# Bissmella/Small-object-detection-transformers

Measured on AMD Instinct MI355X. Metric: images/sec (1024x1024 RGB+IR) train fwd+bwd, higher is better.
Workload: dtype bf16; 1 GPU; SRyolo_MF.yaml (model.yaml graph), batch 8/GPU @ 1024x1024 RGB+IR, fwd + hand-written bwd + fused SGD-nesterov/weight-decay + EMA step, loss = YOLOv5 ComputeLoss (CIoU + BCE, device kernels), 32 synthetic boxes/image, random-init weights; global_batch=8, parallelism=dp1

## Files before the change

small-object-detection-transformers_amd/csrc/head.hip:

```cpp
#include "common.h"
#include "../../include/sodt_hip.h"

namespace {

__global__ void bn_finalize_kernel(const double* __restrict__ stats, float* __restrict__ mr, float* __restrict__ rmean,
                                   float* __restrict__ rvar, long count, int C, float eps, float momentum) {
  const int c = blockIdx.x * blockDim.x + threadIdx.x;
  if (c >= C) return;
  if (stats) {
    double s1 = 0.0, s2 = 0.0;
    for (int r = 0; r < SODT_STATS_REPL; ++r) { s1 += stats[(size_t)r * 2 * C + c]; s2 += stats[(size_t)r * 2 * C + C + c]; }
    const double mean = s1 / (double)count;
    double var = s2 / (double)count - mean * mean;
    if (var < 0.0) var = 0.0;
    mr[c] = (float)mean;
    mr[C + c] = (float)(1.0 / sqrt(var + (double)eps));
    if (rmean) {
      const double unb = count > 1 ? var * (double)count / (double)(count - 1) : var;
      rmean[c] = (1.0f - momentum) * rmean[c] + momentum * (float)mean;
      rvar[c] = (1.0f - momentum) * rvar[c] + momentum * (float)unb;
    }
  } else {
    mr[c] = rmean[c];
    mr[C + c] = rsqrtf(rvar[c] + eps);
  }
}

__global__ void bn_affine_kernel(const float* __restrict__ mr, const float* __restrict__ gamma,
                                 const float* __restrict__ beta, float* __restrict__ scale, float* __restrict__ shift, int C) {
  const int c = blockIdx.x * blockDim.x + threadIdx.x;
  if (c >= C) return;
  const float s = gamma[c] * mr[C + c];
  scale[c] = s;
  shift[c] = beta[c] - mr[c] * s;
}

template <typename T>
__global__ __launch_bounds__(256) void bn_silu_fwd_kernel(const T* __restrict__ z, const float* __restrict__ mr,
                                                         const float* __restrict__ gamma, const float* __restrict__ beta,
                                                         T* __restrict__ y, int ldy, long M, int C) {
  constexpr int KPL = TT<T>::KPL;
  const int CH = C / KPL;
  const long total = M * CH;
  for (long i = (long)blockIdx.x * 256 + threadIdx.x; i < total; i += (long)gridDim.x * 256) {
    const long m = i / CH; const int c0 = (int)(i - m * CH) * KPL;
    float v[KPL];
    unpack<T>(*(const uint4*)(z + m * C + c0), v);
#pragma unroll
    for (int j = 0; j < KPL; ++j) {
      const int c = c0 + j;
      const float a = (v[j] - mr[c]) * mr[C + c] * gamma[c] + beta[c];
      v[j] = a * sigmoid_f(a);
    }
    *(uint4*)(y + m * ldy + c0) = pack<T>(v);
  }
}

template <typename T>
__global__ __launch_bounds__(256) void col_stats_kernel(const T* __restrict__ z, int ldz, double* __restrict__ stats, long M, int C) {
  constexpr int KPL = TT<T>::KPL;
  __shared__ float sred[2][256 * KPL];
  const int CH = C / KPL;
  const int rpp = 256 / CH;
  const int tid = threadIdx.x;
  const int rl = tid / CH, ch = tid - rl * CH;
  const bool act = rl < rpp;
  const int c0 = ch * KPL;
  float a0[KPL], a1[KPL];
#pragma unroll
  for (int j = 0; j < KPL; ++j) { a0[j] = 0.f; a1[j] = 0.f; }
  if (act) {
    const long stride = (long)gridDim.x * rpp;
    for (long m = (long)blockIdx.x * rpp + rl; m < M; m += 4 * stride) {
      uint4 vq[4];
#pragma unroll
      for (int u = 0; u < 4; ++u) {
        const long mm = m + u * stride;
        vq[u] = mm < M ? *(const uint4*)(z + mm * ldz + c0) : make_uint4(0u, 0u, 0u, 0u);
      }
#pragma unroll
      for (int u = 0; u < 4; ++u) {
        float v[KPL];
        unpack<T>(vq[u], v);
#pragma unroll
        for (int j = 0; j < KPL; ++j) { a0[j] += v[j]; a1[j] = fmaf(v[j], v[j], a1[j]); }
      }
    }
  }
#pragma unroll
  for (int j = 0; j < KPL; ++j) { sred[0][tid * KPL + j] = a0[j]; sred[1][tid * KPL + j] = a1[j]; }
  __syncthreads();
  double* st = stats + (size_t)(blockIdx.x % SODT_STATS_REPL) * 2 * C;
  for (int c = tid; c < C; c += 256) {
    const int cc = c / KPL, j = c - cc * KPL;
    double s0 = 0.0, s1 = 0.0;
    for (int r = 0; r < rpp; ++r) { s0 += sred[0][(r * CH + cc) * KPL + j]; s1 += sred[1][(r * CH + cc) * KPL + j]; }
    atomicAdd(st + c, s0);
    atomicAdd(st + C + c, s1);
  }
}

template <typename T>
__global__ __launch_bounds__(256) void bn_silu_bwd_reduce_kernel(const T* __restrict__ dy, int lddy, const T* __restrict__ z,
                                                                const float* __restrict__ mr, const float* __restrict__ gamma,
                                                                const float* __restrict__ beta, double* __restrict__ red,
                                                                long M, int C) {
  constexpr int KPL = TT<T>::KPL;
  __shared__ float sred[2][256 * KPL];
  const int CH = C / KPL;
  const int rpp = 256 / CH;
  const int tid = threadIdx.x;
  const int rl = tid / CH, ch = tid - rl * CH;
  const bool act = rl < rpp;
  const int c0 = ch * KPL;
  float mu[KPL], rs[KPL], ga[KPL], be[KPL], a0[KPL], a1[KPL];
#pragma unroll
  for (int j = 0; j < KPL; ++j) {
    const int c = act ? c0 + j : 0;
    mu[j] = mr[c]; rs[j] = mr[C + c]; ga[j] = gamma[c]; be[j] = beta[c]; a0[j] = 0.f; a1[j] = 0.f;
  }
  if (act) {
    const long stride = (long)gridDim.x * rpp;
    for (long m = (long)blockIdx.x * rpp + rl; m < M; m += 4 * stride) {
      uint4 dq[4], vq[4];
#pragma unroll
      for (int u = 0; u < 4; ++u) {
        const long mm = m + u * stride;
        const bool ok = mm < M;
        dq[u] = ok ? *(const uint4*)(dy + mm * lddy + c0) : make_uint4(0u, 0u, 0u, 0u);
        vq[u] = ok ? *(const uint4*)(z + mm * C + c0) : make_uint4(0u, 0u, 0u, 0u);
      }
#pragma unroll
      for (int u = 0; u < 4; ++u) {
        float d[KPL], v[KPL];
        unpack<T>(dq[u], d);
        unpack<T>(vq[u], v);
#pragma unroll
        for (int j = 0; j < KPL; ++j) {
          const float xh = (v[j] - mu[j]) * rs[j];
          const float a = xh * ga[j] + be[j];
          const float sg = sigmoid_f(a);
          const float gg = d[j] * sg * (1.0f + a * (1.0f - sg));
          a0[j] += gg; a1[j] += gg * xh;
        }
      }
    }
  }
#pragma unroll
  for (int j = 0; j < KPL; ++j) { sred[0][tid * KPL + j] = a0[j]; sred[1][tid * KPL + j] = a1[j]; }
  __syncthreads();
  for (int c = tid; c < C; c += 256) {
    const int cc = c / KPL, j = c - cc * KPL;
    double s0 = 0.0, s1 = 0.0;
    for (int r = 0; r < rpp; ++r) { s0 += sred[0][(r * CH + cc) * KPL + j]; s1 += sred[1][(r * CH + cc) * KPL + j]; }
    atomicAdd(red + c, s0);
    atomicAdd(red + C + c, s1);
  }
}

template <typename T>
__global__ __launch_bounds__(256) void bn_silu_bwd_apply_kernel(const T* __restrict__ dy, int lddy, const T* __restrict__ z,
                                                               const float* __restrict__ mr, const float* __restrict__ gamma,
                                                               const float* __restrict__ beta, const double* __restrict__ red,
                                                               T* __restrict__ dz, float* __restrict__ dgamma,
                                                               float* __restrict__ dbeta, long M, int C) {
  constexpr int KPL = TT<T>::KPL;
  const int CH = C / KPL;
  const long total = M * CH;
  const double invM = 1.0 / (double)M;
  if (blockIdx.x == 0) {
    for (int c = threadIdx.x; c < C; c += 256) { dbeta[c] += (float)red[c]; dgamma[c] += (float)red[C + c]; }
  }
  for (long i = (long)blockIdx.x * 256 + threadIdx.x; i < total; i += (long)gridDim.x * 256) {
    const long m = i / CH; const int c0 = (int)(i - m * CH) * KPL;
    float d[KPL], v[KPL], o[KPL];
    unpack<T>(*(const uint4*)(dy + m * lddy + c0), d);
    unpack<T>(*(const uint4*)(z + m * C + c0), v);
#pragma unroll
    for (int j = 0; j < KPL; ++j) {
      const int c = c0 + j;
      const float rs = mr[C + c], ga = gamma[c];
      const float xh = (v[j] - mr[c]) * rs;
      const float a = xh * ga + beta[c];
      const float sg = sigmoid_f(a);
      const float gg = d[j] * sg * (1.0f + a * (1.0f - sg));
      const float mg = (float)(red[c] * invM), mgx = (float)(red[C + c] * invM);
      o[j] = ga * rs * (gg - mg - xh * mgx);
    }
    *(uint4*)(dz + m * C + c0) = pack<T>(o);
  }
}

template <typename T>
__global__ __launch_bounds__(256) void copy_rows_kernel(const T* __restrict__ src, int lds_, T* __restrict__ dst, int ldd,
                                                       int B, int Ho, int Wo, int shr, int C) {
  constexpr int KPL = TT<T>::KPL;
  const int CH = C / KPL;
  const long total = (long)B * Ho * Wo * CH;
  const int Hi = Ho >> shr, Wi = Wo >> shr;
  for (long i = (long)blockIdx.x * 256 + threadIdx.x; i < total; i += (long)gridDim.x * 256) {
    const long m = i / CH; const int c0 = (int)(i - m * CH) * KPL;
    const int b = (int)(m / ((long)Ho * Wo)); const int rem = (int)(m - (long)b * Ho * Wo);
    const int y = rem / Wo, x = rem - y * Wo;
    const long sm = ((long)b * Hi + (y >> shr)) * Wi + (x >> shr);
    *(uint4*)(dst + m * ldd + c0) = *(const uint4*)(src + sm * lds_ + c0);
  }
}

template <typename T>
__global__ __launch_bounds__(256) void gather_sum_rows_kernel(const T* __restrict__ d, int ldd, T* __restrict__ dsrc, int lds_,
                                                             int B, int Hs, int Ws, int shr, int C, int accumulate) {
  constexpr int KPL = TT<T>::KPL;
  const int CH = C / KPL;
  const long total = (long)B * Hs * Ws * CH;
  const int f = 1 << shr;
  const int Hd = Hs << shr, Wd = Ws << shr;
  for (long i = (long)blockIdx.x * 256 + threadIdx.x; i < total; i += (long)gridDim.x * 256) {
    const long m = i / CH; const int c0 = (int)(i - m * CH) * KPL;
    const int b = (int)(m / ((long)Hs * Ws)); const int rem = (int)(m - (long)b * Hs * Ws);
    const int y = rem / Ws, x = rem - y * Ws;
    float acc[KPL];
#pragma unroll
    for (int j = 0; j < KPL; ++j) acc[j] = 0.f;
    if (accumulate) unpack<T>(*(const uint4*)(dsrc + m * lds_ + c0), acc);
    for (int a = 0; a < f; ++a)
      for (int bb = 0; bb < f; ++bb) {
        const long dm = ((long)b * Hd + (y << shr) + a) * Wd + (x << shr) + bb;
        float v[KPL];
        unpack<T>(*(const uint4*)(d + dm * ldd + c0), v);
#pragma unroll
        for (int j = 0; j < KPL; ++j) acc[j] += v[j];
      }
    *(uint4*)(dsrc + m * lds_ + c0) = pack<T>(acc);
  }
}

template <typename T>
__global__ __launch_bounds__(256) void detect_unpermute_kernel(const float* __restrict__ dpred, T* __restrict__ dz, int ldz,
                                                              int B, int HW, int na, int no) {
  const long total = (long)B * HW * ldz;
  for (long i = (long)blockIdx.x * 256 + threadIdx.x; i < total; i += (long)gridDim.x * 256) {
    const long m = i / ldz; const int n = (int)(i - m * ldz);
    float v = 0.f;
    if (n < na * no) {
      const long b = m / HW, p = m - b * HW;
      const int a = n / no, o = n - a * no;
      v = dpred[((b * na + a) * HW + p) * no + o];
    }
    dz[i] = from_f<T>(v);
  }
}

__global__ __launch_bounds__(256) void detect_decode_kernel(const float* __restrict__ raw, const float* __restrict__ anchor_grid,
                                                           float* __restrict__ zout, int B, int na, int ny, int nx, int no,
                                                           float stride) {
  const long total = (long)B * na * ny * nx * no;
  for (long i = (long)blockIdx.x * 256 + threadIdx.x; i < total; i += (long)gridDim.x * 256) {
    const int o = (int)(i % no); long r = i / no;
    const int x = (int)(r % nx); r /= nx;
    const int y = (int)(r % ny); r /= ny;
    const int a = (int)(r % na);
    const float s = sigmoid_f(raw[i]);
    float v = s;
    if (o == 0) v = (s * 2.f - 0.5f + (float)x) * stride;
    else if (o == 1) v = (s * 2.f - 0.5f + (float)y) * stride;
    else if (o == 2) v = (s * 2.f) * (s * 2.f) * anchor_grid[a * 2];
    else if (o == 3) v = (s * 2.f) * (s * 2.f) * anchor_grid[a * 2 + 1];
    zout[i] = v;
  }
}

template <typename T>
__global__ __launch_bounds__(256) void prep_kernel(const sodt_prep_desc* __restrict__ tab, int n) {
  const sodt_prep_desc d = tab[blockIdx.y];
  const int dims[3] = {d.d0, d.d1, d.d2};
  const int sstr[3] = {d.d1 * d.d2, d.d2, 1};
  const int e0 = dims[d.p0], e1 = dims[d.p1], e2 = dims[d.p2];
  const long total = (long)e0 * e1 * e2;
  T* dst = (T*)d.dst;
  if (d.d2 == 1 && d.p0 == 1 && d.p2 == 0) {
    __shared__ float tile[32][33];
    const int N = d.d0, K = d.d1;
    const int tn = (N + 31) >> 5, tk = (K + 31) >> 5;
    const int tx = threadIdx.x & 31, ty = threadIdx.x >> 5;
    for (int tIdx = blockIdx.x; tIdx < tn * tk; tIdx += gridDim.x) {
      const int n0 = (tIdx / tk) << 5, k0 = (tIdx % tk) << 5;
#pragma unroll
      for (int j = 0; j < 4; ++j) {
        const int n = n0 + ty + 8 * j, k = k0 + tx;
        tile[ty + 8 * j][tx] = (n < N && k < K) ? d.src[(long)n * K + k] : 0.f;
      }
      __syncthreads();
#pragma unroll
      for (int j = 0; j < 4; ++j) {
        const int k = k0 + ty + 8 * j, n = n0 + tx;
        if (k < K && n < N) dst[(long)k * d.dst_ld + n] = from_f<T>(tile[tx][ty + 8 * j]);
      }
      __syncthreads();
    }
    return;
  }
  for (long i = (long)blockIdx.x * 256 + threadIdx.x; i < total; i += (long)gridDim.x * 256) {
    const int i2 = (int)(i % e2); const long r = i / e2;
    const int i1 = (int)(r % e1); const int i0 = (int)(r / e1);
    const long s = (long)i0 * sstr[d.p0] + (long)i1 * sstr[d.p1] + (long)i2 * sstr[d.p2];
    dst[(long)i0 * d.dst_ld + (long)i1 * (d.inner_ld > 0 ? d.inner_ld : e2) + i2] = from_f<T>(d.src[s]);
  }
}

__global__ __launch_bounds__(256) void transpose_f32_kernel(const float* __restrict__ src, float* __restrict__ dst, int rows,
                                                           int cols, int accumulate) {
  const long total = (long)rows * cols;
  for (long i = (long)blockIdx.x * 256 + threadIdx.x; i < total; i += (long)gridDim.x * 256) {
    const int r = (int)(i / cols), c = (int)(i - (long)r * cols);
    if (accumulate) dst[(long)c * rows + r] += src[i];
    else dst[(long)c * rows + r] = src[i];
    if (accumulate == 2) const_cast<float*>(src)[i] = 0.f;
  }
}

template <typename S, typename D>
__global__ __launch_bounds__(256) void cast_kernel(const S* __restrict__ s, D* __restrict__ d, long n) {
  for (long i = (long)blockIdx.x * 256 + threadIdx.x; i < n; i += (long)gridDim.x * 256) d[i] = from_f<D>(to_f(s[i]));
}

template <typename T>
__global__ __launch_bounds__(256) void batch_sum_kernel(const T* __restrict__ d, float* __restrict__ out, int B, long RC) {
  constexpr int KPL = TT<T>::KPL;
  if ((RC % KPL) == 0 && ((uintptr_t)d & 15) == 0 && ((uintptr_t)out & 15) == 0) {
    const long nch = RC / KPL;
    for (long c = (long)blockIdx.x * 256 + threadIdx.x; c < nch; c += (long)gridDim.x * 256) {
      float s[KPL];
#pragma unroll
      for (int j = 0; j < KPL; ++j) s[j] = 0.f;
      for (int b = 0; b < B; ++b) {
        float f[KPL];
        unpack<T>(*(const uint4*)(d + (long)b * RC + c * KPL), f);
#pragma unroll
        for (int j = 0; j < KPL; ++j) s[j] += f[j];
      }
#pragma unroll
      for (int j = 0; j < KPL; j += 4) {
        float4 o = *(float4*)(out + c * KPL + j);
        o.x += s[j]; o.y += s[j + 1]; o.z += s[j + 2]; o.w += s[j + 3];
        *(float4*)(out + c * KPL + j) = o;
      }
    }
    return;
  }
  for (long i = (long)blockIdx.x * 256 + threadIdx.x; i < RC; i += (long)gridDim.x * 256) {
    float s = 0.f;
    for (int b = 0; b < B; ++b) s += to_f(d[(long)b * RC + i]);
    out[i] += s;
  }
}

inline unsigned nblocks(long work, int cap = 4096) {
  long b = (work + 255) / 256;
  if (b < 1) b = 1;
  if (b > cap) b = cap;
  return (unsigned)b;
}

}

extern "C" int sodt_bn_finalize(const double* stats, float* mean_rstd, float* running_mean, float* running_var,
                                long count, int C, float eps, float momentum, sodt_stream_t st) {
  if (!mean_rstd || C <= 0 || (!stats && (!running_mean || !running_var))) return SODT_EINVAL;
  hipLaunchKernelGGL(bn_finalize_kernel, dim3((C + 255) / 256), dim3(256), 0, (hipStream_t)st, stats, mean_rstd,
                     running_mean, running_var, count, C, eps, momentum);
  return hipGetLastError() == hipSuccess ? SODT_OK : SODT_EINVAL;
}

extern "C" int sodt_bn_affine(const float* mean_rstd, const float* gamma, const float* beta, float* scale, float* shift,
                              int C, sodt_stream_t st) {
  if (!mean_rstd || !gamma || !beta || !scale || !shift || C <= 0) return SODT_EINVAL;
  hipLaunchKernelGGL(bn_affine_kernel, dim3((C + 255) / 256), dim3(256), 0, (hipStream_t)st, mean_rstd, gamma, beta, scale, shift, C);
  return hipGetLastError() == hipSuccess ? SODT_OK : SODT_EINVAL;
}

extern "C" int sodt_bn_silu_fwd(const void* z, const float* mean_rstd, const float* gamma, const float* beta,
                                void* y, int ldy, long M, int C, int dtype, sodt_stream_t st) {
  const int kpl = dtype == SODT_BF16 ? 8 : 4;
  if (!z || !y || M <= 0 || C <= 0 || (C % kpl) || (ldy % kpl)) return SODT_EINVAL;
  const unsigned gr = nblocks(M * (C / kpl));
  if (dtype == SODT_BF16) hipLaunchKernelGGL(bn_silu_fwd_kernel<bf16>, dim3(gr), dim3(256), 0, (hipStream_t)st, (const bf16*)z, mean_rstd, gamma, beta, (bf16*)y, ldy, M, C);
  else if (dtype == SODT_F32) hipLaunchKernelGGL(bn_silu_fwd_kernel<float>, dim3(gr), dim3(256), 0, (hipStream_t)st, (const float*)z, mean_rstd, gamma, beta, (float*)y, ldy, M, C);
  else return SODT_EINVAL;
  return hipGetLastError() == hipSuccess ? SODT_OK : SODT_EINVAL;
}

extern "C" int sodt_bn_silu_bwd_reduce(const void* dy, int lddy, const void* z, const float* mean_rstd,
                                       const float* gamma, const float* beta, double* red, long M, int C,
                                       int dtype, sodt_stream_t st) {
  const int kpl = dtype == SODT_BF16 ? 8 : 4;
  if (!dy || !z || !red || M <= 0 || C <= 0 || (C % kpl) || (lddy % kpl) || C / kpl > 256) return SODT_EINVAL;
  const int rpp = 256 / (C / kpl);
  long gr = (M + rpp - 1) / rpp; if (gr > 1024) gr = 1024;
  if (dtype == SODT_BF16) hipLaunchKernelGGL(bn_silu_bwd_reduce_kernel<bf16>, dim3((unsigned)gr), dim3(256), 0, (hipStream_t)st, (const bf16*)dy, lddy, (const bf16*)z, mean_rstd, gamma, beta, red, M, C);
  else if (dtype == SODT_F32) hipLaunchKernelGGL(bn_silu_bwd_reduce_kernel<float>, dim3((unsigned)gr), dim3(256), 0, (hipStream_t)st, (const float*)dy, lddy, (const float*)z, mean_rstd, gamma, beta, red, M, C);
  else return SODT_EINVAL;
  return hipGetLastError() == hipSuccess ? SODT_OK : SODT_EINVAL;
}

extern "C" int sodt_col_stats(const void* z, int ldz, double* stats, long M, int C, int dtype, sodt_stream_t st) {
  const int kpl = dtype == SODT_BF16 ? 8 : 4;
  if (!z || !stats || M <= 0 || C <= 0 || (C % kpl) || (ldz % kpl) || C / kpl > 256 || (((uintptr_t)z) & 15)) return SODT_EINVAL;
  const int rpp = 256 / (C / kpl);
  long gr = (M + 4L * rpp - 1) / (4L * rpp); if (gr > 1024) gr = 1024;
  if (dtype == SODT_BF16) hipLaunchKernelGGL(col_stats_kernel<bf16>, dim3((unsigned)gr), dim3(256), 0, (hipStream_t)st, (const bf16*)z, ldz, stats, M, C);
  else if (dtype == SODT_F32) hipLaunchKernelGGL(col_stats_kernel<float>, dim3((unsigned)gr), dim3(256), 0, (hipStream_t)st, (const float*)z, ldz, stats, M, C);
  else return SODT_EINVAL;
  return hipGetLastError() == hipSuccess ? SODT_OK : SODT_EINVAL;
}

extern "C" int sodt_bn_silu_bwd_apply(const void* dy, int lddy, const void* z, const float* mean_rstd,
                                      const float* gamma, const float* beta, const double* red, void* dz,
                                      float* dgamma, float* dbeta, long M, int C, int dtype, sodt_stream_t st) {
  const int kpl = dtype == SODT_BF16 ? 8 : 4;
  if (!dy || !z || !red || !dz || !dgamma || !dbeta || M <= 0 || C <= 0 || (C % kpl) || (lddy % kpl)) return SODT_EINVAL;
  const unsigned gr = nblocks(M * (C / kpl));
  if (dtype == SODT_BF16) hipLaunchKernelGGL(bn_silu_bwd_apply_kernel<bf16>, dim3(gr), dim3(256), 0, (hipStream_t)st, (const bf16*)dy, lddy, (const bf16*)z, mean_rstd, gamma, beta, red, (bf16*)dz, dgamma, dbeta, M, C);
  else if (dtype == SODT_F32) hipLaunchKernelGGL(bn_silu_bwd_apply_kernel<float>, dim3(gr), dim3(256), 0, (hipStream_t)st, (const float*)dy, lddy, (const float*)z, mean_rstd, gamma, beta, red, (float*)dz, dgamma, dbeta, M, C);
  else return SODT_EINVAL;
  return hipGetLastError() == hipSuccess ? SODT_OK : SODT_EINVAL;
}

extern "C" int sodt_copy_rows(const void* src, int lds_, void* dst, int ldd, int B, int Ho, int Wo, int shr, int C,
                              int dtype, sodt_stream_t st) {
  const int kpl = dtype == SODT_BF16 ? 8 : 4;
  if (!src || !dst || B <= 0 || Ho <= 0 || Wo <= 0 || shr < 0 || C <= 0 || (C % kpl) || (lds_ % kpl) || (ldd % kpl)) return SODT_EINVAL;
  if ((Ho & ((1 << shr) - 1)) || (Wo & ((1 << shr) - 1))) return SODT_EINVAL;
  const unsigned gr = nblocks((long)B * Ho * Wo * (C / kpl));
  if (dtype == SODT_BF16) hipLaunchKernelGGL(copy_rows_kernel<bf16>, dim3(gr), dim3(256), 0, (hipStream_t)st, (const bf16*)src, lds_, (bf16*)dst, ldd, B, Ho, Wo, shr, C);
  else if (dtype == SODT_F32) hipLaunchKernelGGL(copy_rows_kernel<float>, dim3(gr), dim3(256), 0, (hipStream_t)st, (const float*)src, lds_, (float*)dst, ldd, B, Ho, Wo, shr, C);
  else return SODT_EINVAL;
  return hipGetLastError() == hipSuccess ? SODT_OK : SODT_EINVAL;
}

extern "C" int sodt_gather_sum_rows(const void* d, int ldd, void* dsrc, int lds_, int B, int Hs, int Ws, int shr, int C,
                                    int accumulate, int dtype, sodt_stream_t st) {
  const int kpl = dtype == SODT_BF16 ? 8 : 4;
  if (!d || !dsrc || B <= 0 || Hs <= 0 || Ws <= 0 || shr < 0 || C <= 0 || (C % kpl) || (lds_ % kpl) || (ldd % kpl)) return SODT_EINVAL;
  const unsigned gr = nblocks((long)B * Hs * Ws * (C / kpl));
  if (dtype == SODT_BF16) hipLaunchKernelGGL(gather_sum_rows_kernel<bf16>, dim3(gr), dim3(256), 0, (hipStream_t)st, (const bf16*)d, ldd, (bf16*)dsrc, lds_, B, Hs, Ws, shr, C, accumulate);
  else if (dtype == SODT_F32) hipLaunchKernelGGL(gather_sum_rows_kernel<float>, dim3(gr), dim3(256), 0, (hipStream_t)st, (const float*)d, ldd, (float*)dsrc, lds_, B, Hs, Ws, shr, C, accumulate);
  else return SODT_EINVAL;
  return hipGetLastError() == hipSuccess ? SODT_OK : SODT_EINVAL;
}

extern "C" int sodt_detect_unpermute(const float* dpred, void* dz, int ldz, int B, int HW, int na, int no,
                                     int dtype, sodt_stream_t st) {
  if (!dpred || !dz || B <= 0 || HW <= 0 || na * no > ldz) return SODT_EINVAL;
  const unsigned gr = nblocks((long)B * HW * ldz);
  if (dtype == SODT_BF16) hipLaunchKernelGGL(detect_unpermute_kernel<bf16>, dim3(gr), dim3(256), 0, (hipStream_t)st, dpred, (bf16*)dz, ldz, B, HW, na, no);
  else if (dtype == SODT_F32) hipLaunchKernelGGL(detect_unpermute_kernel<float>, dim3(gr), dim3(256), 0, (hipStream_t)st, dpred, (float*)dz, ldz, B, HW, na, no);
  else return SODT_EINVAL;
  return hipGetLastError() == hipSuccess ? SODT_OK : SODT_EINVAL;
}

extern "C" int sodt_detect_decode(const float* raw, const float* anchor_grid, float* z, int B, int na, int ny, int nx,
                                  int no, float stride, sodt_stream_t st) {
  if (!raw || !anchor_grid || !z || B <= 0 || na <= 0 || ny <= 0 || nx <= 0 || no < 5) return SODT_EINVAL;
  hipLaunchKernelGGL(detect_decode_kernel, dim3(nblocks((long)B * na * ny * nx * no)), dim3(256), 0, (hipStream_t)st,
                     raw, anchor_grid, z, B, na, ny, nx, no, stride);
  return hipGetLastError() == hipSuccess ? SODT_OK : SODT_EINVAL;
}

extern "C" int sodt_prep_weights(const sodt_prep_desc* table_dev, int n, int max_elems, int dtype, sodt_stream_t st) {
  if (!table_dev || n <= 0 || max_elems <= 0) return SODT_EINVAL;
  unsigned bx = nblocks(max_elems / 4, 512);
  if (dtype == SODT_BF16) hipLaunchKernelGGL(prep_kernel<bf16>, dim3(bx, n), dim3(256), 0, (hipStream_t)st, table_dev, n);
  else if (dtype == SODT_F32) hipLaunchKernelGGL(prep_kernel<float>, dim3(bx, n), dim3(256), 0, (hipStream_t)st, table_dev, n);
  else return SODT_EINVAL;
  return hipGetLastError() == hipSuccess ? SODT_OK : SODT_EINVAL;
}

extern "C" int sodt_transpose_f32(const float* src, float* dst, int rows, int cols, int accumulate, sodt_stream_t st) {
  if (!src || !dst || rows <= 0 || cols <= 0) return SODT_EINVAL;
  hipLaunchKernelGGL(transpose_f32_kernel, dim3(nblocks((long)rows * cols)), dim3(256), 0, (hipStream_t)st, src, dst, rows, cols, accumulate);
  return hipGetLastError() == hipSuccess ? SODT_OK : SODT_EINVAL;
}

extern "C" int sodt_cast(const void* src, void* dst, long n, int src_dtype, int dst_dtype, sodt_stream_t st) {
  if (!src || !dst || n <= 0) return SODT_EINVAL;
  const unsigned gr = nblocks(n);
  if (src_dtype == SODT_F32 && dst_dtype == SODT_BF16) hipLaunchKernelGGL((cast_kernel<float, bf16>), dim3(gr), dim3(256), 0, (hipStream_t)st, (const float*)src, (bf16*)dst, n);
  else if (src_dtype == SODT_BF16 && dst_dtype == SODT_F32) hipLaunchKernelGGL((cast_kernel<bf16, float>), dim3(gr), dim3(256), 0, (hipStream_t)st, (const bf16*)src, (float*)dst, n);
  else if (src_dtype == SODT_F32 && dst_dtype == SODT_F32) hipLaunchKernelGGL((cast_kernel<float, float>), dim3(gr), dim3(256), 0, (hipStream_t)st, (const float*)src, (float*)dst, n);
  else return SODT_EINVAL;
  return hipGetLastError() == hipSuccess ? SODT_OK : SODT_EINVAL;
}

extern "C" int sodt_batch_sum(const void* d, float* out, int B, long RC, int dtype, sodt_stream_t st) {
  if (!d || !out || B <= 0 || RC <= 0) return SODT_EINVAL;
  const unsigned gr = nblocks(RC / 4);
  if (dtype == SODT_BF16) hipLaunchKernelGGL(batch_sum_kernel<bf16>, dim3(gr), dim3(256), 0, (hipStream_t)st, (const bf16*)d, out, B, RC);
  else if (dtype == SODT_F32) hipLaunchKernelGGL(batch_sum_kernel<float>, dim3(gr), dim3(256), 0, (hipStream_t)st, (const float*)d, out, B, RC);
  else return SODT_EINVAL;
  return hipGetLastError() == hipSuccess ? SODT_OK : SODT_EINVAL;
}

extern "C" int sodt_memset_zero(void* p, long bytes, sodt_stream_t st) {
  if (!p || bytes <= 0) return SODT_EINVAL;
  return hipMemsetAsync(p, 0, (size_t)bytes, (hipStream_t)st) == hipSuccess ? SODT_OK : SODT_EINVAL;
}

extern "C" const char* sodt_version(void) { return "sodt_hip 0.1 (gfx950)"; }
```

small-object-detection-transformers_amd/csrc/norm.hip:

```cpp
#include "common.h"
#include "../../include/sodt_hip.h"

namespace {


template <typename T, int MAXCH>
__global__ __launch_bounds__(256) void ln_fwd_kernel(const T* __restrict__ x, const float* __restrict__ gamma,
                                                     const float* __restrict__ beta, T* __restrict__ y,
                                                     float* __restrict__ stats, int M, int C) {
  constexpr int KPL = TT<T>::KPL;
  const int lane = threadIdx.x & 63, wid = threadIdx.x >> 6;
  const int nch = C / KPL;
  const float invC = 1.0f / (float)C;
  for (long row = (long)blockIdx.x * 4 + wid; row < M; row += (long)gridDim.x * 4) {
    float v[MAXCH][KPL];
    float s = 0.f;
#pragma unroll
    for (int i = 0; i < MAXCH; ++i) {
      const int ch = lane + 64 * i;
      if (ch < nch) {
        unpack<T>(*(const uint4*)(x + row * C + ch * KPL), v[i]);
#pragma unroll
        for (int j = 0; j < KPL; ++j) s += v[i][j];
      }
    }
    const float mean = wave_sum(s) * invC;
    float q = 0.f;
#pragma unroll
    for (int i = 0; i < MAXCH; ++i) {
      const int ch = lane + 64 * i;
      if (ch < nch) {
#pragma unroll
        for (int j = 0; j < KPL; ++j) { const float d = v[i][j] - mean; q += d * d; }
      }
    }
    const float rstd = rsqrtf(wave_sum(q) * invC + 1e-5f);
    if (lane == 0 && stats) { stats[row * 2] = mean; stats[row * 2 + 1] = rstd; }
#pragma unroll
    for (int i = 0; i < MAXCH; ++i) {
      const int ch = lane + 64 * i;
      if (ch < nch) {
        float o[KPL];
#pragma unroll
        for (int j = 0; j < KPL; ++j) o[j] = (v[i][j] - mean) * rstd * gamma[ch * KPL + j] + beta[ch * KPL + j];
        *(uint4*)(y + row * C + ch * KPL) = pack<T>(o);
      }
    }
  }
}

template <typename T, int MAXCH>
__global__ __launch_bounds__(256) void ln_bwd_kernel(const T* __restrict__ dy, const T* __restrict__ x,
                                                     const float* __restrict__ stats, const float* __restrict__ gamma,
                                                     const T* __restrict__ dres, T* __restrict__ dx,
                                                     float* __restrict__ dgamma, float* __restrict__ dbeta,
                                                     int M, int C) {
  constexpr int KPL = TT<T>::KPL;
  __shared__ float red[4][64 * MAXCH * KPL + 1];
  const int lane = threadIdx.x & 63, wid = threadIdx.x >> 6;
  const int nch = C / KPL;
  const float invC = 1.0f / (float)C;
  float ag[MAXCH][KPL], ab[MAXCH][KPL], gm[MAXCH][KPL];
#pragma unroll
  for (int i = 0; i < MAXCH; ++i) {
    const int ch = lane + 64 * i;
#pragma unroll
    for (int j = 0; j < KPL; ++j) {
      ag[i][j] = 0.f; ab[i][j] = 0.f;
      gm[i][j] = (ch < nch) ? gamma[ch * KPL + j] : 0.f;
    }
  }
  for (long row = (long)blockIdx.x * 4 + wid; row < M; row += (long)gridDim.x * 4) {
    const float mean = stats[row * 2], rstd = stats[row * 2 + 1];
    float xh[MAXCH][KPL], g[MAXCH][KPL];
    float c1 = 0.f, c2 = 0.f;
#pragma unroll
    for (int i = 0; i < MAXCH; ++i) {
      const int ch = lane + 64 * i;
      if (ch < nch) {
        float a[KPL], d[KPL];
        unpack<T>(*(const uint4*)(x + row * C + ch * KPL), a);
        unpack<T>(*(const uint4*)(dy + row * C + ch * KPL), d);
#pragma unroll
        for (int j = 0; j < KPL; ++j) {
          xh[i][j] = (a[j] - mean) * rstd;
          g[i][j] = d[j] * gm[i][j];
          c1 += g[i][j]; c2 += g[i][j] * xh[i][j];
          ag[i][j] += d[j] * xh[i][j]; ab[i][j] += d[j];
        }
      }
    }
    c1 = wave_sum(c1) * invC; c2 = wave_sum(c2) * invC;
#pragma unroll
    for (int i = 0; i < MAXCH; ++i) {
      const int ch = lane + 64 * i;
      if (ch < nch) {
        float o[KPL];
#pragma unroll
        for (int j = 0; j < KPL; ++j) o[j] = rstd * (g[i][j] - c1 - xh[i][j] * c2);
        if (dres) {
          float r[KPL];
          unpack<T>(*(const uint4*)(dres + row * C + ch * KPL), r);
#pragma unroll
          for (int j = 0; j < KPL; ++j) o[j] += r[j];
        }
        *(uint4*)(dx + row * C + ch * KPL) = pack<T>(o);
      }
    }
  }
  for (int pass = 0; pass < 2; ++pass) {
    __syncthreads();
#pragma unroll
    for (int i = 0; i < MAXCH; ++i)
#pragma unroll
      for (int j = 0; j < KPL; ++j)
        red[wid][(lane + 64 * i) * KPL + j] = pass == 0 ? ag[i][j] : ab[i][j];
    __syncthreads();
    for (int c = threadIdx.x; c < C; c += 256) {
      const float t = red[0][c] + red[1][c] + red[2][c] + red[3][c];
      atomicAdd((pass == 0 ? dgamma : dbeta) + c, t);
    }
  }
}

__device__ __forceinline__ float half_sum(float v) {
  v += __shfl_xor(v, 1); v += __shfl_xor(v, 2); v += __shfl_xor(v, 4); v += __shfl_xor(v, 8); v += __shfl_xor(v, 16);
  return v;
}

template <typename T>
__global__ __launch_bounds__(256) void ln_fwd_half_kernel(const T* __restrict__ x, const float* __restrict__ gamma,
                                                          const float* __restrict__ beta, T* __restrict__ y,
                                                          float* __restrict__ stats, int M, int C) {
  constexpr int KPL = TT<T>::KPL;
  const int lane = threadIdx.x & 63, wid = threadIdx.x >> 6, l32 = lane & 31, sub = lane >> 5;
  const int nch = C / KPL;
  const bool act = l32 < nch;
  const float invC = 1.0f / (float)C;
  float gm[KPL], bt[KPL];
#pragma unroll
  for (int j = 0; j < KPL; ++j) { gm[j] = act ? gamma[l32 * KPL + j] : 0.f; bt[j] = act ? beta[l32 * KPL + j] : 0.f; }
  for (long row = ((long)blockIdx.x * 4 + wid) * 2 + sub; row < M; row += (long)gridDim.x * 8) {
    float v[KPL];
#pragma unroll
    for (int j = 0; j < KPL; ++j) v[j] = 0.f;
    if (act) unpack<T>(*(const uint4*)(x + row * C + l32 * KPL), v);
    float s = 0.f;
#pragma unroll
    for (int j = 0; j < KPL; ++j) s += v[j];
    const float mean = half_sum(s) * invC;
    float q = 0.f;
    if (act) {
#pragma unroll
      for (int j = 0; j < KPL; ++j) { const float d = v[j] - mean; q += d * d; }
    }
    const float rstd = rsqrtf(half_sum(q) * invC + 1e-5f);
    if (l32 == 0 && stats) { stats[row * 2] = mean; stats[row * 2 + 1] = rstd; }
    if (act) {
      float o[KPL];
#pragma unroll
      for (int j = 0; j < KPL; ++j) o[j] = (v[j] - mean) * rstd * gm[j] + bt[j];
      *(uint4*)(y + row * C + l32 * KPL) = pack<T>(o);
    }
  }
}

template <typename T>
__global__ __launch_bounds__(256) void ln_bwd_half_kernel(const T* __restrict__ dy, const T* __restrict__ x,
                                                          const float* __restrict__ stats, const float* __restrict__ gamma,
                                                          const T* __restrict__ dres, T* __restrict__ dx,
                                                          float* __restrict__ dgamma, float* __restrict__ dbeta,
                                                          int M, int C) {
  constexpr int KPL = TT<T>::KPL;
  __shared__ float red[8][32 * KPL + 1];
  const int lane = threadIdx.x & 63, wid = threadIdx.x >> 6, l32 = lane & 31, sub = lane >> 5;
  const int nch = C / KPL;
  const bool act = l32 < nch;
  const float invC = 1.0f / (float)C;
  float ag[KPL], ab[KPL], gm[KPL];
#pragma unroll
  for (int j = 0; j < KPL; ++j) { ag[j] = 0.f; ab[j] = 0.f; gm[j] = act ? gamma[l32 * KPL + j] : 0.f; }
  for (long row = ((long)blockIdx.x * 4 + wid) * 2 + sub; row < M; row += (long)gridDim.x * 8) {
    const float mean = stats[row * 2], rstd = stats[row * 2 + 1];
    float xh[KPL], g[KPL];
    float c1 = 0.f, c2 = 0.f;
#pragma unroll
    for (int j = 0; j < KPL; ++j) { xh[j] = 0.f; g[j] = 0.f; }
    if (act) {
      float a[KPL], d[KPL];
      unpack<T>(*(const uint4*)(x + row * C + l32 * KPL), a);
      unpack<T>(*(const uint4*)(dy + row * C + l32 * KPL), d);
#pragma unroll
      for (int j = 0; j < KPL; ++j) {
        xh[j] = (a[j] - mean) * rstd;
        g[j] = d[j] * gm[j];
        c1 += g[j]; c2 += g[j] * xh[j];
        ag[j] += d[j] * xh[j]; ab[j] += d[j];
      }
    }
    c1 = half_sum(c1) * invC; c2 = half_sum(c2) * invC;
    if (act) {
      float o[KPL];
#pragma unroll
      for (int j = 0; j < KPL; ++j) o[j] = rstd * (g[j] - c1 - xh[j] * c2);
      if (dres) {
        float r[KPL];
        unpack<T>(*(const uint4*)(dres + row * C + l32 * KPL), r);
#pragma unroll
        for (int j = 0; j < KPL; ++j) o[j] += r[j];
      }
      *(uint4*)(dx + row * C + l32 * KPL) = pack<T>(o);
    }
  }
  for (int pass = 0; pass < 2; ++pass) {
    __syncthreads();
#pragma unroll
    for (int j = 0; j < KPL; ++j) red[wid * 2 + sub][l32 * KPL + j] = pass == 0 ? ag[j] : ab[j];
    __syncthreads();
    for (int c = threadIdx.x; c < C; c += 256) {
      float t = 0.f;
#pragma unroll
      for (int r = 0; r < 8; ++r) t += red[r][c];
      atomicAdd((pass == 0 ? dgamma : dbeta) + c, t);
    }
  }
}

}

extern "C" int sodt_layernorm_fwd(const void* x, const float* gamma, const float* beta, void* y, float* stats,
                                  int M, int C, int dtype, sodt_stream_t st) {
  const int kpl = dtype == SODT_BF16 ? 8 : 4;
  if (M <= 0 || C <= 0 || (C % kpl) || C > 256 * kpl || !x || !y || !gamma || !beta) return SODT_EINVAL;
  long blocks = ((long)M + 3) / 4;
  if (blocks > 4096) blocks = 4096;
  if (C / kpl <= 32) {
    long hb = ((long)M + 7) / 8;
    if (hb > 4096) hb = 4096;
    if (dtype == SODT_BF16) hipLaunchKernelGGL(ln_fwd_half_kernel<bf16>, dim3((unsigned)hb), dim3(256), 0, (hipStream_t)st, (const bf16*)x, gamma, beta, (bf16*)y, stats, M, C);
    else hipLaunchKernelGGL(ln_fwd_half_kernel<float>, dim3((unsigned)hb), dim3(256), 0, (hipStream_t)st, (const float*)x, gamma, beta, (float*)y, stats, M, C);
    return hipGetLastError() == hipSuccess ? SODT_OK : SODT_EINVAL;
  }
  const int nc = (C / kpl + 63) / 64;
#define LNF(TY, NC) hipLaunchKernelGGL((ln_fwd_kernel<TY, NC>), dim3((unsigned)blocks), dim3(256), 0, (hipStream_t)st, \
                       (const TY*)x, gamma, beta, (TY*)y, stats, M, C)
  if (dtype == SODT_BF16) { if (nc == 1) LNF(bf16, 1); else if (nc == 2) LNF(bf16, 2); else LNF(bf16, 4); }
  else { if (nc == 1) LNF(float, 1); else if (nc == 2) LNF(float, 2); else LNF(float, 4); }
#undef LNF
  return hipGetLastError() == hipSuccess ? SODT_OK : SODT_EINVAL;
}

extern "C" int sodt_layernorm_bwd(const void* dy, const void* x, const float* stats, const float* gamma,
                                  const void* dres, void* dx, float* dgamma, float* dbeta,
                                  int M, int C, int dtype, sodt_stream_t st) {
  const int kpl = dtype == SODT_BF16 ? 8 : 4;
  if (M <= 0 || C <= 0 || (C % kpl) || C > 256 * kpl || !x || !dy || !dx || !stats || !gamma || !dgamma || !dbeta)
    return SODT_EINVAL;
  long blocks = ((long)M + 3) / 4;
  if (blocks > 1024) blocks = 1024;
  if (C / kpl <= 32) {
    long hb = ((long)M + 7) / 8;
    if (hb > 1024) hb = 1024;
    if (dtype == SODT_BF16) hipLaunchKernelGGL(ln_bwd_half_kernel<bf16>, dim3((unsigned)hb), dim3(256), 0, (hipStream_t)st, (const bf16*)dy, (const bf16*)x, stats, gamma, (const bf16*)dres, (bf16*)dx, dgamma, dbeta, M, C);
    else hipLaunchKernelGGL(ln_bwd_half_kernel<float>, dim3((unsigned)hb), dim3(256), 0, (hipStream_t)st, (const float*)dy, (const float*)x, stats, gamma, (const float*)dres, (float*)dx, dgamma, dbeta, M, C);
    return hipGetLastError() == hipSuccess ? SODT_OK : SODT_EINVAL;
  }
  const int nc = (C / kpl + 63) / 64;
#define LNB(TY, NC) hipLaunchKernelGGL((ln_bwd_kernel<TY, NC>), dim3((unsigned)blocks), dim3(256), 0, (hipStream_t)st, \
                       (const TY*)dy, (const TY*)x, stats, gamma, (const TY*)dres, (TY*)dx, dgamma, dbeta, M, C)
  if (dtype == SODT_BF16) { if (nc == 1) LNB(bf16, 1); else if (nc == 2) LNB(bf16, 2); else LNB(bf16, 4); }
  else { if (nc == 1) LNB(float, 1); else if (nc == 2) LNB(float, 2); else LNB(float, 4); }
#undef LNB
  return hipGetLastError() == hipSuccess ? SODT_OK : SODT_EINVAL;
}
```

Measured before the change: 211.1 images/sec.

## Add row-tiled BN-SiLU forward and LN backward kernels, tune BN reduce grid

Adds a BN+SiLU forward kernel that assigns fixed channel slices per thread, hoists per-channel mean/rstd/gamma/beta into registers and processes several rows per iteration, used instead of the flat-index kernel when the channel count packs well. The BN-SiLU backward reduce now unrolls eight rows per iteration with a smaller capped grid, and replaces its serial per-channel shared-memory sum with a tree reduction before the double atomics. Adds an LN backward variant for mid-sized C that batches four rows per wave to issue more loads ahead of use. These target memory latency, per-element index division and atomic traffic, at the cost of higher register pressure and fewer blocks.

```diff
diff --git a/small-object-detection-transformers_amd/csrc/head.hip b/small-object-detection-transformers_amd/csrc/head.hip
--- a/small-object-detection-transformers_amd/csrc/head.hip
+++ b/small-object-detection-transformers_amd/csrc/head.hip
@@ -56,6 +56,54 @@
   }
 }
 
+constexpr int BN_ROWS_U = 4;
+#ifndef BN_ROWS_CAP
+#define BN_ROWS_CAP 2048
+#endif
+constexpr int BN_RED_U = 8;
+#ifndef BN_RED_CAP
+#define BN_RED_CAP 256
+#endif
+
+template <typename T>
+__global__ __launch_bounds__(256) void bn_silu_fwd_rows_kernel(const T* __restrict__ z, const float* __restrict__ mr,
+                                                              const float* __restrict__ gamma, const float* __restrict__ beta,
+                                                              T* __restrict__ y, int ldy, long M, int C) {
+  constexpr int KPL = TT<T>::KPL;
+  const int CH = C / KPL;
+  const int rpp = 256 / CH;
+  const int tid = threadIdx.x;
+  const int rl = tid / CH, ch = tid - rl * CH;
+  if (rl >= rpp) return;
+  const int c0 = ch * KPL;
+  float mu[KPL], rs[KPL], ga[KPL], be[KPL];
+#pragma unroll
+  for (int j = 0; j < KPL; ++j) { mu[j] = mr[c0 + j]; rs[j] = mr[C + c0 + j]; ga[j] = gamma[c0 + j]; be[j] = beta[c0 + j]; }
+  const long stride = (long)gridDim.x * rpp;
+  for (long m = (long)blockIdx.x * rpp + rl; m < M; m += BN_ROWS_U * stride) {
+    uint4 vq[BN_ROWS_U];
+#pragma unroll
+    for (int u = 0; u < BN_ROWS_U; ++u) {
+      const long mm = m + u * stride;
+      vq[u] = mm < M ? *(const uint4*)(z + mm * C + c0) : make_uint4(0u, 0u, 0u, 0u);
+    }
+#pragma unroll
+    for (int u = 0; u < BN_ROWS_U; ++u) {
+      const long mm = m + u * stride;
+      if (mm < M) {
+        float v[KPL];
+        unpack<T>(vq[u], v);
+#pragma unroll
+        for (int j = 0; j < KPL; ++j) {
+          const float a = (v[j] - mu[j]) * rs[j] * ga[j] + be[j];
+          v[j] = a * sigmoid_f(a);
+        }
+        *(uint4*)(y + mm * ldy + c0) = pack<T>(v);
+      }
+    }
+  }
+}
+
 template <typename T>
 __global__ __launch_bounds__(256) void col_stats_kernel(const T* __restrict__ z, int ldz, double* __restrict__ stats, long M, int C) {
   constexpr int KPL = TT<T>::KPL;
@@ -121,17 +169,17 @@
   }
   if (act) {
     const long stride = (long)gridDim.x * rpp;
-    for (long m = (long)blockIdx.x * rpp + rl; m < M; m += 4 * stride) {
-      uint4 dq[4], vq[4];
-#pragma unroll
-      for (int u = 0; u < 4; ++u) {
+    for (long m = (long)blockIdx.x * rpp + rl; m < M; m += BN_RED_U * stride) {
+      uint4 dq[BN_RED_U], vq[BN_RED_U];
+#pragma unroll
+      for (int u = 0; u < BN_RED_U; ++u) {
         const long mm = m + u * stride;
         const bool ok = mm < M;
         dq[u] = ok ? *(const uint4*)(dy + mm * lddy + c0) : make_uint4(0u, 0u, 0u, 0u);
         vq[u] = ok ? *(const uint4*)(z + mm * C + c0) : make_uint4(0u, 0u, 0u, 0u);
       }
 #pragma unroll
-      for (int u = 0; u < 4; ++u) {
+      for (int u = 0; u < BN_RED_U; ++u) {
         float d[KPL], v[KPL];
         unpack<T>(dq[u], d);
         unpack<T>(vq[u], v);
@@ -149,12 +197,21 @@
 #pragma unroll
   for (int j = 0; j < KPL; ++j) { sred[0][tid * KPL + j] = a0[j]; sred[1][tid * KPL + j] = a1[j]; }
   __syncthreads();
+  int s = 1;
+  while (s < rpp) s <<= 1;
+  for (s >>= 1; s >= 1; s >>= 1) {
+    if (act && rl < s && rl + s < rpp) {
+#pragma unroll
+      for (int j = 0; j < KPL; ++j) {
+        sred[0][tid * KPL + j] += sred[0][(tid + s * CH) * KPL + j];
+        sred[1][tid * KPL + j] += sred[1][(tid + s * CH) * KPL + j];
+      }
+    }
+    __syncthreads();
+  }
   for (int c = tid; c < C; c += 256) {
-    const int cc = c / KPL, j = c - cc * KPL;
-    double s0 = 0.0, s1 = 0.0;
-    for (int r = 0; r < rpp; ++r) { s0 += sred[0][(r * CH + cc) * KPL + j]; s1 += sred[1][(r * CH + cc) * KPL + j]; }
-    atomicAdd(red + c, s0);
-    atomicAdd(red + C + c, s1);
+    atomicAdd(red + c, (double)sred[0][c]);
+    atomicAdd(red + C + c, (double)sred[1][c]);
   }
 }
 
@@ -362,6 +419,14 @@
   return (unsigned)b;
 }
 
+inline bool bn_rows_ok(int ch) { return ch <= 256 && (256 / ch) * ch >= 224; }
+inline unsigned bn_rows_grid(long M, int ch, int u, int cap) {
+  const long per = (long)u * (256 / ch);
+  long b = (M + per - 1) / per;
+  if (b > cap) b = cap;
+  return (unsigned)b;
+}
+
 }
 
 extern "C" int sodt_bn_finalize(const double* stats, float* mean_rstd, float* running_mean, float* running_var,
@@ -383,6 +448,13 @@
                                 void* y, int ldy, long M, int C, int dtype, sodt_stream_t st) {
   const int kpl = dtype == SODT_BF16 ? 8 : 4;
   if (!z || !y || M <= 0 || C <= 0 || (C % kpl) || (ldy % kpl)) return SODT_EINVAL;
+  if (dtype != SODT_BF16 && dtype != SODT_F32) return SODT_EINVAL;
+  if (bn_rows_ok(C / kpl)) {
+    const unsigned gw = bn_rows_grid(M, C / kpl, BN_ROWS_U, BN_ROWS_CAP);
+    if (dtype == SODT_BF16) hipLaunchKernelGGL(bn_silu_fwd_rows_kernel<bf16>, dim3(gw), dim3(256), 0, (hipStream_t)st, (const bf16*)z, mean_rstd, gamma, beta, (bf16*)y, ldy, M, C);
+    else hipLaunchKernelGGL(bn_silu_fwd_rows_kernel<float>, dim3(gw), dim3(256), 0, (hipStream_t)st, (const float*)z, mean_rstd, gamma, beta, (float*)y, ldy, M, C);
+    return hipGetLastError() == hipSuccess ? SODT_OK : SODT_EINVAL;
+  }
   const unsigned gr = nblocks(M * (C / kpl));
   if (dtype == SODT_BF16) hipLaunchKernelGGL(bn_silu_fwd_kernel<bf16>, dim3(gr), dim3(256), 0, (hipStream_t)st, (const bf16*)z, mean_rstd, gamma, beta, (bf16*)y, ldy, M, C);
   else if (dtype == SODT_F32) hipLaunchKernelGGL(bn_silu_fwd_kernel<float>, dim3(gr), dim3(256), 0, (hipStream_t)st, (const float*)z, mean_rstd, gamma, beta, (float*)y, ldy, M, C);
@@ -395,8 +467,7 @@
                                        int dtype, sodt_stream_t st) {
   const int kpl = dtype == SODT_BF16 ? 8 : 4;
   if (!dy || !z || !red || M <= 0 || C <= 0 || (C % kpl) || (lddy % kpl) || C / kpl > 256) return SODT_EINVAL;
-  const int rpp = 256 / (C / kpl);
-  long gr = (M + rpp - 1) / rpp; if (gr > 1024) gr = 1024;
+  const unsigned gr = bn_rows_grid(M, C / kpl, BN_RED_U, BN_RED_CAP);
   if (dtype == SODT_BF16) hipLaunchKernelGGL(bn_silu_bwd_reduce_kernel<bf16>, dim3((unsigned)gr), dim3(256), 0, (hipStream_t)st, (const bf16*)dy, lddy, (const bf16*)z, mean_rstd, gamma, beta, red, M, C);
   else if (dtype == SODT_F32) hipLaunchKernelGGL(bn_silu_bwd_reduce_kernel<float>, dim3((unsigned)gr), dim3(256), 0, (hipStream_t)st, (const float*)dy, lddy, (const float*)z, mean_rstd, gamma, beta, red, M, C);
   else return SODT_EINVAL;
diff --git a/small-object-detection-transformers_amd/csrc/norm.hip b/small-object-detection-transformers_amd/csrc/norm.hip
--- a/small-object-detection-transformers_amd/csrc/norm.hip
+++ b/small-object-detection-transformers_amd/csrc/norm.hip
@@ -3,6 +3,9 @@
 
 namespace {
 
+#ifndef LN_BWD_CAP
+#define LN_BWD_CAP 512
+#endif
 
 template <typename T, int MAXCH>
 __global__ __launch_bounds__(256) void ln_fwd_kernel(const T* __restrict__ x, const float* __restrict__ gamma,
@@ -105,6 +108,103 @@
           for (int j = 0; j < KPL; ++j) o[j] += r[j];
         }
         *(uint4*)(dx + row * C + ch * KPL) = pack<T>(o);
+      }
+    }
+  }
+  for (int pass = 0; pass < 2; ++pass) {
+    __syncthreads();
+#pragma unroll
+    for (int i = 0; i < MAXCH; ++i)
+#pragma unroll
+      for (int j = 0; j < KPL; ++j)
+        red[wid][(lane + 64 * i) * KPL + j] = pass == 0 ? ag[i][j] : ab[i][j];
+    __syncthreads();
+    for (int c = threadIdx.x; c < C; c += 256) {
+      const float t = red[0][c] + red[1][c] + red[2][c] + red[3][c];
+      atomicAdd((pass == 0 ? dgamma : dbeta) + c, t);
+    }
+  }
+}
+
+template <typename T, int MAXCH, int R>
+__global__ __launch_bounds__(256) void ln_bwd_rows_kernel(const T* __restrict__ dy, const T* __restrict__ x,
+                                                     const float* __restrict__ stats, const float* __restrict__ gamma,
+                                                     const T* __restrict__ dres, T* __restrict__ dx,
+                                                     float* __restrict__ dgamma, float* __restrict__ dbeta,
+                                                     int M, int C) {
+  constexpr int KPL = TT<T>::KPL;
+  __shared__ float red[4][64 * MAXCH * KPL + 1];
+  const int lane = threadIdx.x & 63, wid = threadIdx.x >> 6;
+  const int nch = C / KPL;
+  const float invC = 1.0f / (float)C;
+  float ag[MAXCH][KPL], ab[MAXCH][KPL], gm[MAXCH][KPL];
+#pragma unroll
+  for (int i = 0; i < MAXCH; ++i) {
+    const int ch = lane + 64 * i;
+#pragma unroll
+    for (int j = 0; j < KPL; ++j) {
+      ag[i][j] = 0.f; ab[i][j] = 0.f;
+      gm[i][j] = (ch < nch) ? gamma[ch * KPL + j] : 0.f;
+    }
+  }
+  const long wstride = (long)gridDim.x * 4;
+  for (long row0 = (long)blockIdx.x * 4 + wid; row0 < M; row0 += R * wstride) {
+    uint4 xq[R][MAXCH], dq[R][MAXCH], rq[R][MAXCH];
+    float mean[R], rstd[R];
+#pragma unroll
+    for (int r = 0; r < R; ++r) {
+      const long row = row0 + r * wstride;
+      const bool rok = row < M;
+      mean[r] = rok ? stats[row * 2] : 0.f;
+      rstd[r] = rok ? stats[row * 2 + 1] : 0.f;
+#pragma unroll
+      for (int i = 0; i < MAXCH; ++i) {
+        const int ch = lane + 64 * i;
+        const bool ok = rok && ch < nch;
+        xq[r][i] = ok ? *(const uint4*)(x + row * C + ch * KPL) : make_uint4(0u, 0u, 0u, 0u);
+        dq[r][i] = ok ? *(const uint4*)(dy + row * C + ch * KPL) : make_uint4(0u, 0u, 0u, 0u);
+        rq[r][i] = (ok && dres) ? *(const uint4*)(dres + row * C + ch * KPL) : make_uint4(0u, 0u, 0u, 0u);
+      }
+    }
+#pragma unroll
+    for (int r = 0; r < R; ++r) {
+      const long row = row0 + r * wstride;
+      if (row < M) {
+        float xh[MAXCH][KPL], g[MAXCH][KPL];
+        float c1 = 0.f, c2 = 0.f;
+#pragma unroll
+        for (int i = 0; i < MAXCH; ++i) {
+          const int ch = lane + 64 * i;
+          if (ch < nch) {
+            float a[KPL], d[KPL];
+            unpack<T>(xq[r][i], a);
+            unpack<T>(dq[r][i], d);
+#pragma unroll
+            for (int j = 0; j < KPL; ++j) {
+              xh[i][j] = (a[j] - mean[r]) * rstd[r];
+              g[i][j] = d[j] * gm[i][j];
+              c1 += g[i][j]; c2 += g[i][j] * xh[i][j];
+              ag[i][j] += d[j] * xh[i][j]; ab[i][j] += d[j];
+            }
+          }
+        }
+        c1 = wave_sum(c1) * invC; c2 = wave_sum(c2) * invC;
+#pragma unroll
+        for (int i = 0; i < MAXCH; ++i) {
+          const int ch = lane + 64 * i;
+          if (ch < nch) {
+            float o[KPL];
+#pragma unroll
+            for (int j = 0; j < KPL; ++j) o[j] = rstd[r] * (g[i][j] - c1 - xh[i][j] * c2);
+            if (dres) {
+              float rr[KPL];
+              unpack<T>(rq[r][i], rr);
+#pragma unroll
+              for (int j = 0; j < KPL; ++j) o[j] += rr[j];
+            }
+            *(uint4*)(dx + row * C + ch * KPL) = pack<T>(o);
+          }
+        }
       }
     }
   }
@@ -266,6 +366,13 @@
     return hipGetLastError() == hipSuccess ? SODT_OK : SODT_EINVAL;
   }
   const int nc = (C / kpl + 63) / 64;
+  if (nc == 2) {
+    long rb = ((long)M + 15) / 16;
+    if (rb > LN_BWD_CAP) rb = LN_BWD_CAP;
+    if (dtype == SODT_BF16) hipLaunchKernelGGL((ln_bwd_rows_kernel<bf16, 2, 4>), dim3((unsigned)rb), dim3(256), 0, (hipStream_t)st, (const bf16*)dy, (const bf16*)x, stats, gamma, (const bf16*)dres, (bf16*)dx, dgamma, dbeta, M, C);
+    else hipLaunchKernelGGL((ln_bwd_rows_kernel<float, 2, 4>), dim3((unsigned)rb), dim3(256), 0, (hipStream_t)st, (const float*)dy, (const float*)x, stats, gamma, (const float*)dres, (float*)dx, dgamma, dbeta, M, C);
+    return hipGetLastError() == hipSuccess ? SODT_OK : SODT_EINVAL;
+  }
 #define LNB(TY, NC) hipLaunchKernelGGL((ln_bwd_kernel<TY, NC>), dim3((unsigned)blocks), dim3(256), 0, (hipStream_t)st, \
                        (const TY*)dy, (const TY*)x, stats, gamma, (const TY*)dres, (TY*)dx, dgamma, dbeta, M, C)
   if (dtype == SODT_BF16) { if (nc == 1) LNB(bf16, 1); else if (nc == 2) LNB(bf16, 2); else LNB(bf16, 4); }
```

Measured after the change: 212.9 images/sec (median of 6 runs). Within noise of the previous version (+0.9%).
